# pangsu0613/TransCAR

Measured on AMD Instinct MI355X. Metric: nuScenes frames/sec (6-cam+radar, 900 queries): fusion decoder (Detr3DHead.forward + box decode), FPN features resident in HBM, higher is better.
Workload: dtype f32 (linear steps and attention core of the batched launches: f16x2 split operands, 3 v_mfma_f32_16x16x32_f16 products, fp32 accumulate; activations of the 32-row tiles held as two f16 planes; 4- / 8-row tiles: f32 MFMA)

## Files before the change

### transcar_amd/csrc/chain.hip

```cpp
#include <stdlib.h>
#include <string.h>

#include <type_traits>

#include "kernels.hpp"
#ifdef TC_CHAIN_STAMPS
__device__ long long g_cam_stamps[4][8];
#define CAM_STAMP(slot)                                                                        \
  do {                                                                                         \
    if (blockIdx.x == 100 && (threadIdx.x & 63) == 0)                                          \
      g_cam_stamps[(threadIdx.x >> 6) & 3][(slot)] = __builtin_amdgcn_s_memtime();             \
  } while (0)
#endif
#include "rowdev.hpp"
#define TC_ONCE_LD(p) ldg4_stream(p)
#ifdef TC_CHAIN_DUMP
__device__ float* g_chain_dump;
__device__ long long g_chain_dump_floats;
#endif

namespace tc {

namespace {

// ... 76 lines not shown
  F_CARRY = 4096,
  F_NOT_LAYER0 = 8192,
  F_PRESYNC = 16384
};
enum GSel : short {
  G_NONE = -1, G_HS = 0, G_QK, G_VT, G_INITREF, G_ATTN_O, G_XIN, G_POS, G_CLS, G_KV0, G_KV1, G_KV2,
  G_QF, G_RFEAT, G_COUNT
};

struct StepDesc {
  short kind, wp, wp2, K, N, src, src2, dst, res, act, flags, gsel, gtsel, sync;
};
constexpr StepDesc PROG_DECODER_T[] = {
    {K_LOAD, 0, 0, 0, 0, B_NONE, B_NONE, B_U1, B_NONE, 0, 0, G_ATTN_O, G_NONE, 0},
    {K_LOAD, 0, 0, 0, 0, B_NONE, B_NONE, B_X, B_NONE, 0, 0, G_XIN, G_NONE, 1},
    {K_LINEAR, 1, -1, 256, 256, B_U1, B_NONE, B_U2, B_X, 0, 0, G_NONE, G_NONE, 1},
    {K_LN, 2, -1, 0, 0, B_U2, B_NONE, B_X, B_U1, 0, F_LN_XP, G_NONE, G_NONE, 1},
    {K_LINEAR, 3, -1, 256, N_LOGITS, B_U1, B_NONE, B_L, B_NONE, 0, 0, G_NONE, G_NONE, 0},
    {K_POSENC, 5, 6, 0, 0, B_NONE, B_NONE, B_U2, B_NONE, 0, F_NOT_W0, G_NONE, G_NONE, 1},
    {K_SAMPLE, 0, 0, 0, 0, B_L, B_NONE, B_U3, B_NONE, 0, 0, G_NONE, G_NONE, 1},
    {K_LINEAR, 7, -1, 256, 256, B_U2, B_NONE, B_U1, B_NONE, 0, 0, G_NONE, G_NONE, 1},
    {K_LINEAR, 4, -1, 256, 256, B_U3, B_NONE, B_U2, B_X, 0, 0, G_NONE, G_NONE, 1},
    {K_LN, 9, 8, 0, 0, B_U2, B_U1, B_X, B_NONE, 0, 0, G_NONE, G_NONE, 1},
    {K_LINEAR, 10, -1, 256, 512, B_X, B_NONE, B_A, B_NONE, 1, 0, G_NONE, G_NONE, 1},
    {K_LINEAR, 11, -1, 512, 256, B_A, B_NONE, B_U3, B_X, 0, 0, G_NONE, G_NONE, 1},
    {K_LN, 12, -1, 0, 0, B_U3, B_NONE, B_X, B_U1, 0, F_LN_XP, G_HS, G_NONE, 1},
    {K_LINEAR, 13, -1, 256, 256, B_X, B_NONE, B_U2, B_NONE, 1, 0, G_NONE, G_NONE, 0},
    {K_LINEAR, 16, -1, 256, 512, B_U1, B_NONE, B_NONE, B_NONE, 0, F_SCALEQ | F_SKIP_NONEXT, G_QK, G_NONE, 0},
    {K_LINEAR, 16, -1, 256, 256, B_X, B_NONE, B_NONE, B_NONE, 0, F_WOFF | F_SKIP_NONEXT, G_NONE, G_VT, 1},
    {K_LINEAR, 14, -1, 256, 256, B_U2, B_NONE, B_U3, B_NONE, 1, 0, G_NONE, G_NONE, 0},
    {K_NARROW, 15, -1, 256, N_CODE, B_U3, B_U1, B_L, B_NONE, 0, F_PRESYNC, G_NONE, G_NONE, 1},
    {K_REFUPD, 0, 0, 0, 0, B_L, B_NONE, B_NONE, B_NONE, 0, 0, G_NONE, G_NONE, 0},
    {K_END, 0, 0, 0, 0, 0, 0, 0, 0, 0, 0, 0, 0, 0}};
constexpr StepDesc PROG_PROLOGUE_T[] = {
    {K_LOAD, 0, 0, 0, 0, B_NONE, B_NONE, B_U1, B_NONE, 0, 0, G_POS, G_NONE, 0},
    {K_LOAD, 0, 0, 0, 0, B_NONE, B_NONE, B_X, B_NONE, 0, 0, G_XIN, G_NONE, 1},
    {K_LINEAR, 0, -1, 256, 3, B_U1, B_NONE, B_NONE, B_NONE, 2, 0, G_INITREF, G_NONE, 0},
    {K_LINEAR, 16, -1, 256, 512, B_X, B_U1, B_NONE, B_NONE, 0, F_SCALEQ, G_QK, G_NONE, 0},
    {K_LINEAR, 16, -1, 256, 256, B_X, B_NONE, B_NONE, B_NONE, 0, F_WOFF, G_NONE, G_VT, 0},
    {K_END, 0, 0, 0, 0, 0, 0, 0, 0, 0, 0, 0, 0, 0}};
constexpr StepDesc PROG_RADAR_ENC_T[] = {
    {K_TOKENS, 0, 0, 0, 0, B_NONE, B_NONE, B_A, B_NONE, 0, 0, G_NONE, G_NONE, 1},
    {K_POSENC, 0, 1, 0, 0, B_A, B_NONE, B_U3, B_NONE, 0, 0, G_NONE, G_NONE, 0},
    {K_LINEAR, 4, -1, 36, 64, B_A, B_NONE, B_X, B_NONE, 1, 0, G_NONE, G_NONE, 1},
    {K_LINEAR, 2, -1, 256, 256, B_U3, B_NONE, B_U1, B_NONE, 0, 0, G_NONE, G_NONE, 0},
    {K_LINEAR, 5, -1, 64, 128, B_X, B_NONE, B_U2, B_NONE, 1, 0, G_NONE, G_NONE, 1},
    {K_LINEAR, 6, -1, 128, 256, B_U2, B_NONE, B_X, B_NONE, 1, 0, G_NONE, G_NONE, 1},
    {K_LN, 3, -1, 0, 0, B_U1, B_NONE, B_U2, B_X, 0, F_LN_RELU, G_NONE, G_NONE, 1},
    {K_LINEAR, 7, -1, 256, 512, B_U2, B_NONE, B_NONE, B_NONE, 0, 0, G_KV0, G_NONE, 0},
    {K_LINEAR, 8, -1, 256, 512, B_U2, B_NONE, B_NONE, B_NONE, 0, 0, G_KV1, G_NONE, 0},
    {K_LINEAR, 9, -1, 256, 512, B_U2, B_NONE, B_NONE, B_NONE, 0, 0, G_KV2, G_NONE, 0},
    {K_END, 0, 0, 0, 0, 0, 0, 0, 0, 0, 0, 0, 0, 0}};
constexpr StepDesc PROG_RADAR_ENC_A_T[] = {
    {K_TOKENS, 0, 0, 0, 0, B_NONE, B_NONE, B_A, B_NONE, 0, 0, G_NONE, G_NONE, 1},
    {K_POSENC, 0, 1, 0, 0, B_A, B_NONE, B_U3, B_NONE, 0, 0, G_NONE, G_NONE, 0},
    {K_LINEAR, 4, -1, 36, 64, B_A, B_NONE, B_X, B_NONE, 1, 0, G_NONE, G_NONE, 1},
    {K_LINEAR, 2, -1, 256, 256, B_U3, B_NONE, B_U1, B_NONE, 0, 0, G_NONE, G_NONE, 0},
    {K_LINEAR, 5, -1, 64, 128, B_X, B_NONE, B_U2, B_NONE, 1, 0, G_NONE, G_NONE, 1},
    {K_LINEAR, 6, -1, 128, 256, B_U2, B_NONE, B_X, B_NONE, 1, 0, G_NONE, G_NONE, 1},
    {K_LN, 3, -1, 0, 0, B_U1, B_NONE, B_U2, B_X, 0, F_LN_RELU, G_RFEAT, G_NONE, 1},
    {K_LINEAR, 7, -1, 256, 512, B_U2, B_NONE, B_NONE, B_NONE, 0, 0, G_KV0, G_NONE, 0},
    {K_END, 0, 0, 0, 0, 0, 0, 0, 0, 0, 0, 0, 0, 0}};
constexpr StepDesc PROG_RADAR_ENC_B_T[] = {
    {K_LOAD, 0, 0, 0, 0, B_NONE, B_NONE, B_X, B_NONE, 0, 0, G_RFEAT, G_NONE, 1},
    {K_LINEAR, 8, -1, 256, 512, B_X, B_NONE, B_NONE, B_NONE, 0, 0, G_KV1, G_NONE, 0},
    {K_LINEAR, 9, -1, 256, 512, B_X, B_NONE, B_NONE, B_NONE, 0, 0, G_KV2, G_NONE, 0},
// ... 67 lines not shown
  float qscale; int qpad;
  DropK drop;
  int dbg;
  int tile_rows;
  int matrix_path;
  int last_cls_only;
  const float* ref_in; int ref_mod; float* ref_out; float* box_m;
  CamK cam; unsigned long long* pair_counter;
  const float* pre; const int* premask;
  const float* tokens; int RI, T, pad_mult;
  const float* ref_last; const float* box_in;
  int cen_from_box;
  float rmin[TC_MAX_RADAR_LAYERS], rmax[TC_MAX_RADAR_LAYERS];
  float* all_box; int* hits;
  const int* row_perm;
  float* tape[T_COUNT]; size_t tape_stride; size_t hits_stride;
  DropK rdrop;
  const float* bwd_cxy[TC_MAX_RADAR_LAYERS]; int bwd_ldc[TC_MAX_RADAR_LAYERS];
  const float* bwd_box[TC_MAX_RADAR_LAYERS];
  int* range_status;
  const float* loss_vals;
  float* loss_out;
  const DetAcc* detp;
};
struct ChainK : ChainDev {
  tc_linear pairs[MAX_PAIRS];
  tc_linear gpairs[MAX_PAIRS];
  float* dy[D_COUNT]; size_t dy_stride = 0;
  const float* d_cls = nullptr; const float* d_box = nullptr;
  float* dkv[TC_MAX_RADAR_LAYERS] = {nullptr, nullptr, nullptr};
  size_t w16_delta = 0;
  int npoints = 1;
  int refine = 1;
};

inline bool generic_xattn(const ChainK& k) { return k.npoints > 1 || k.cam.num_levels < 4; }

constexpr int table_steps(int prog) {
  return (prog == PROG_DECODER ? (int)(sizeof(PROG_DECODER_T) / sizeof(StepDesc))
          : prog == PROG_PROLOGUE ? (int)(sizeof(PROG_PROLOGUE_T) / sizeof(StepDesc))
          : prog_is_enc_full(prog) ? (int)(sizeof(PROG_RADAR_ENC_T) / sizeof(StepDesc))
          : prog == PROG_RADAR_ENC_A ? (int)(sizeof(PROG_RADAR_ENC_A_T) / sizeof(StepDesc))
          : prog == PROG_RADAR_ENC_B ? (int)(sizeof(PROG_RADAR_ENC_B_T) / sizeof(StepDesc))
          : prog == PROG_RADAR_BWD ? (int)(sizeof(PROG_RADAR_BWD_T) / sizeof(StepDesc))
                                     : (int)(sizeof(PROG_RADAR_LAYER_T) / sizeof(StepDesc))) - 1;
}
constexpr int rec_cap(int prog) { return table_steps(prog) * ((prog_is_radar(prog) || prog == PROG_RADAR_BWD) ? TC_MAX_RADAR_LAYERS : 1); }
static_assert(sizeof(BWD_STORE) / sizeof(short) == table_steps(PROG_RADAR_BWD), "backward maps follow the step table");
static_assert(sizeof(RADAR_TAPE) / sizeof(short) == table_steps(PROG_RADAR) && sizeof(ENC_TAPE) / sizeof(short) == table_steps(PROG_RADAR_ENC),
              "tape maps follow the step tables");
inline const StepDesc* prog_table(int prog) {
  return prog == PROG_DECODER ? PROG_DECODER_T
         : prog == PROG_PROLOGUE ? PROG_PROLOGUE_T
         : prog_is_enc_full(prog) ? PROG_RADAR_ENC_T
         : prog == PROG_RADAR_ENC_A ? PROG_RADAR_ENC_A_T
         : prog == PROG_RADAR_ENC_B ? PROG_RADAR_ENC_B_T
         : prog == PROG_RADAR_BWD ? PROG_RADAR_BWD_T : PROG_RADAR_LAYER_T;
}

struct LinSpec {
  const float* W; const float* bias; int K, N;
  const float* src; int src_ld;
  const float* src2; int src2_ld;
  float* dst; int dst_ld;
  const float* res; int res_ld;
  const int* gate;
// ... 1852 lines not shown
}

template <int RA, int RB, int PROGB, int MM = 0, bool PRE = false, bool MP = false>
__global__ __launch_bounds__(nw_of(RA) * 64, 2) void chain_dual_kernel(ChainDev ka, ChainDev kb, int na,
                                                           Recs<rec_cap(PROG_DECODER), nw_of(RA)> ra,
                                                           Recs<rec_cap(PROGB), nw_of(RB)> rb) {
  static_assert(nw_of(RA) == nw_of(RB), "both programs of a launch run with the same workgroup size");
  if ((int)blockIdx.x < na) chain_body<RA, PROG_DECODER, false, MM, PRE, MP>(ka, ra.s, blockIdx.x);
  else chain_body<RB, PROGB, false, MM>(kb, rb.s, (int)blockIdx.x - na);
}

template <int R, int PROG>
int lds_off(int id) {
  using Lds = ChainLds<R, rec_cap(PROG)>;
  const int unit0 = (int)(offsetof(Lds, unit) / 4), ustride = R * LD2;
  switch (id) {
    case B_A: return unit0 + ustride;
    case B_X: return unit0;
    case B_U1: return unit0 + ustride;
    case B_U2: return unit0 + 2 * ustride;
    case B_U3: return unit0 + 3 * ustride;
    case B_L: return (int)(offsetof(Lds, l) / 4);
    default: return -1;
  }
}
template <int R, int PROG>
constexpr size_t chain_lds_bytes() { return sizeof(ChainLds<R, rec_cap(PROG)>); }
inline int buf_ld_h(int id) { return id == B_A ? LD5 : id == B_L ? LDL : LD2; }

template <int R, int PROG, int MM = 0>
void resolve_program(ChainK& k, StepAllT<nw_of(R)>* out) {
  constexpr int NW = nw_of(R);
  const StepDesc* table = prog_table(PROG);
  constexpr int nsteps = table_steps(PROG);
  const int nrep = (prog_is_radar(PROG) || PROG == PROG_RADAR_BWD) ? k.nlayers : 1;
  const int total = nsteps * nrep;
  memset(out, 0, sizeof(StepAllT<NW>) * rec_cap(PROG));
  for (int idx = 0; idx < total; ++idx) {
    const int rep = idx / nsteps, si = idx - rep * nsteps;
    const int layer = PROG == PROG_RADAR_BWD ? k.nlayers - 1 - rep : rep;
    const int pair0 = (prog_is_radar(PROG) || PROG == PROG_RADAR_BWD) ? layer * RADAR_PAIRS : 0;
    const StepDesc d = table[si];
    StepRes& r = out[idx].r;
    r.K = d.K; r.N = d.N;
    r.kind = d.kind; r.src = d.src; r.src2 = d.src2; r.dst = d.dst; r.res = d.res; r.act = d.act;
    r.flags = d.flags; r.sync = d.sync; r.rep = (short)rep; r.si = (short)si;
    if ((d.flags & F_SKIP_NONEXT) && !k.has_next) r.kind = K_NOP;
    if (PROG == PROG_DECODER && !k.refine &&
        (d.kind == K_REFUPD || ((d.kind == K_LINEAR || d.kind == K_NARROW) && d.wp >= 13 && d.wp <= 15)))
      r.kind = K_NOP;
    if (PROG == PROG_RADAR && k.last_cls_only && rep + 1 < nrep && d.wp >= 6 && d.wp <= 10 &&
        (d.kind == K_LINEAR || d.kind == K_LN || d.kind == K_NARROW))
      r.kind = K_NOP;
    if (d.gsel != G_NONE) { r.gd = k.g[d.gsel]; r.gld = k.g_ld[d.gsel]; r.gmod = k.g_mod[d.gsel]; }
    if (d.gtsel != G_NONE) r.gt = k.g[d.gtsel];
    bool taped = false;
    if (PROG == PROG_RADAR_TRAIN) {
      if (d.flags & F_SCALEQ) r.flags = (short)(r.flags & ~F_SCALEQ);
      r.flags = (short)(r.flags & ~F_IFHIT);
      if (d.kind == K_LINEAR && d.wp == 4) r.flags = (short)(r.flags | F_GPRE);
      const short ts = RADAR_TAPE[si];
      if (ts != T_NONE && r.gd == nullptr) { r.gd = k.tape[ts] + (size_t)rep * k.tape_stride; r.gld = 256; taped = true; }
    }
    if (PROG == PROG_RADAR_BWD) {
      if ((d.flags & F_NOT_LAYER0) && layer == 0) r.kind = K_NOP;
      const short ds = BWD_STORE[si], ts = BWD_TAPE[si], ts2 = BWD_TAPE2[si];
      if (ds != D_NONE && k.dy[ds] != nullptr) { r.gd = k.dy[ds] + (size_t)layer * k.dy_stride; taped = true; }
// ... 279 lines not shown
  const tc_decoder_layer& w = *a.w;
  const tc_pos_encoder& pe = w.position_encoder;
  k.pairs[0] = w.self_attn.in_proj; k.pairs[1] = w.self_attn.out_proj;
  k.pairs[2] = tc_linear{w.norm0.g, w.norm0.b};
  k.pairs[3] = w.attention_weights; k.pairs[4] = w.output_proj; k.pairs[5] = pe.l0;
  k.pairs[6] = tc_linear{pe.n1.g, pe.n1.b}; k.pairs[7] = pe.l3; k.pairs[8] = tc_linear{pe.n4.g, pe.n4.b};
  k.pairs[9] = tc_linear{w.norm1.g, w.norm1.b}; k.pairs[10] = w.ffn0; k.pairs[11] = w.ffn1;
  k.pairs[12] = tc_linear{w.norm2.g, w.norm2.b};
  k.pairs[13] = w.reg.l0; k.pairs[14] = w.reg.l2; k.pairs[15] = w.reg.l4;
  k.refine = w.reg.l0.w != nullptr;
  TC_REQUIRE(k.refine || a.box_m == nullptr, "decoder_chain: a layer without a reg branch writes no box");
  k.has_next = a.next_in_proj != nullptr;
  if (k.has_next) k.pairs[16] = *a.next_in_proj;
  k.w16_delta = w.packed16_delta;
  k.g[G_ATTN_O] = const_cast<float*>(a.attn_o); k.g_ld[G_ATTN_O] = 256; k.g_mod[G_ATTN_O] = a.attn_mod;
  k.g[G_XIN] = const_cast<float*>(a.x_in); k.g_ld[G_XIN] = a.x_ld; k.g_mod[G_XIN] = a.x_mod;
  k.g[G_POS] = const_cast<float*>(a.qe); k.g_ld[G_POS] = 512; k.g_mod[G_POS] = a.Q;
  k.g[G_HS] = a.hs; k.g_ld[G_HS] = 256;
  k.g[G_QK] = a.qk; k.g_ld[G_QK] = 512; k.g[G_VT] = a.vt;
  k.qscale = a.qscale; k.qpad = a.qpad;
  k.ref_in = a.ref_in; k.ref_mod = a.ref_mod; k.ref_out = a.ref_out; k.box_m = a.box_m;
  fill_camk(a.cam, k.cam);
  k.pair_counter = a.cam.pair_counter;
  TC_REQUIRE((a.pre == nullptr) == (a.premask == nullptr), "decoder_chain: pre-gathered values and masks come together");
  TC_REQUIRE(a.pre == nullptr || a.cam.feats.num_levels == 4,
             "decoder_chain: num_levels=%d (the camera pre-gather exists for 4 levels)", a.cam.feats.num_levels);
  k.pre = a.pre; k.premask = a.premask;
  TC_REQUIRE(a.tile_rows == 0 || a.tile_rows == 4 || a.tile_rows == 8 || a.tile_rows == 16 || a.tile_rows == 32,
             "decoder_chain: tile_rows=%d (0 = automatic, 4, 8, 16 or 32)", a.tile_rows);
  k.tile_rows = a.tile_rows;
  k.matrix_path = a.matrix_path;
  k.drop = a.drop;
  k.range_status = a.range_status;
  return 0;
}

int launch_decoder_chain(const DecoderChainArgs& a, hipStream_t s) {
  ChainK k;
  int rc = make_decoder_k(a, k);
  if (rc != 0) return rc;
  return launch(k, s, "chain(decoder)");
}

static int make_radar_enc_k(const RadarEncodeArgs& a, ChainK& k, int part = 0) {
  TC_REQUIRE(a.RI <= 64 && (a.RI & 3) == 0, "radar_encode: radar_in_dims=%d", a.RI);
  TC_REQUIRE(a.nlayers == TC_MAX_RADAR_LAYERS, "radar_encode: %d radar layers (3 supported)", a.nlayers);
  init_k(k);
  k.program = part == 1 ? PROG_RADAR_ENC_A : part == 2 ? PROG_RADAR_ENC_B : PROG_RADAR_ENC;
  if (a.tape != nullptr) {
    TC_REQUIRE(part == 0, "radar_encode: the training forward runs the whole encoder program");
    k.program = PROG_RADAR_ENC_TRAIN;
    for (int i = 0; i < T_COUNT; ++i) k.tape[i] = a.tape[i];
  }
  k.M = a.M; k.Q = 1; k.RI = a.RI; k.tokens = a.tokens; k.has_next = 1;
  k.w16_delta = a.w16_delta; k.matrix_path = a.matrix_path; k.range_status = a.range_status;
  TC_REQUIRE(part == 0 || a.radar_feat != nullptr, "radar_encode: split programs need the radar_feat buffer");
  k.g[G_RFEAT] = a.radar_feat; k.g_ld[G_RFEAT] = 256;
  k.pairs[0] = a.rpe.l0; k.pairs[1] = tc_linear{a.rpe.n1.g, a.rpe.n1.b}; k.pairs[2] = a.rpe.l3;
  k.pairs[3] = tc_linear{a.rpe.n4.g, a.rpe.n4.b}; k.pairs[4] = a.f0; k.pairs[5] = a.f2; k.pairs[6] = a.f4;
  for (int r = 0; r < TC_MAX_RADAR_LAYERS; ++r) {
    k.pairs[7 + r] = a.kvproj[r];
    k.g[G_KV0 + r] = a.kv[r]; k.g_ld[G_KV0 + r] = 512;
  }
  return 0;
}

int launch_radar_encode(const RadarEncodeArgs& a, hipStream_t s) {
// ... 215 lines not shown
```

### transcar_amd/csrc/head.hip

```cpp
#include <math.h>
#include <stdarg.h>
#include <stdlib.h>
#include <string.h>

#include "kernels.hpp"

namespace tc {

static thread_local char g_err[512] = "";

void set_error(const char* fmt, ...) {
  va_list ap;
  va_start(ap, fmt);
  vsnprintf(g_err, sizeof(g_err), fmt, ap);
  va_end(ap);
}

int check_launch(const char* what) {
  hipError_t e = hipGetLastError();
  if (e != hipSuccess) {
    set_error("%s: %s", what, hipGetErrorString(e));
    return (int)e;
  }
  return 0;
// ... 110 lines not shown
};

static size_t head_ws_layout(const tc_head_weights* w, int B, int T, void* base, size_t cap,
                             HeadWs* out) {
  const int Q = w->num_query, C = w->embed_dims, F = w->ffn_dims, L = w->num_layers;
  const size_t rows = (size_t)B * Q, rt = (size_t)B * T;
  const int qpad = ((Q + 15) / 16) * 16;
  Arena a(base, cap);
  HeadWs h;
  h.qpad = qpad;
  h.pos = a.take<float>(rows * C); h.x = a.take<float>(rows * C);
  h.qk = a.take<float>(rows * 2 * C); h.vt = a.take<float>((size_t)B * C * qpad);
  h.attn_o = a.take<float>(rows * C);
  h.t0 = a.take<float>(rows * C); h.t1 = a.take<float>(rows * C); h.t2 = a.take<float>(rows * C);
  h.ffn_h = a.take<float>(rows * F);
  h.logits = a.take<float>(rows * w->num_cams * w->num_levels * head_points(w));
  h.sampled = a.take<float>(rows * C);
  h.init_ref = a.take<float>(rows * 3); h.inter_refs = a.take<float>((size_t)L * rows * 3);
  h.hs = a.take<float>((size_t)L * rows * C);
  h.reg_tmp = a.take<float>(rows * w->code_size); h.box_m = a.take<float>(rows * w->code_size);
  h.tp0 = a.take<float>(rt * C); h.tp1 = a.take<float>(rt * C);
  h.f0 = a.take<float>(rt * 64); h.f1 = a.take<float>(rt * 128); h.f2 = a.take<float>(rt * C);
  h.radar_feat = a.take<float>(rt * C); h.kv = a.take<float>(rt * 2 * C);
  for (int i = 0; i < TC_MAX_RADAR_LAYERS; ++i) h.kv3[i] = a.take<float>(rt * 2 * C);
  h.qproj = a.take<float>(rows * C); h.rattn = a.take<float>(rows * C);
  h.cxy = a.take<float>(rows * 2); h.addref = a.take<float>(rows * 3);
  h.qf = a.take<float>(rows * C);
  h.hits = a.take<int>((size_t)TC_MAX_RADAR_LAYERS * rows);
  h.perm = a.take<int>(rows); h.hitflag = a.take<int>(rows);
  if (out) *out = h;
  return a.off;
}

static int head_forward_fused(const tc_head_weights* w, const tc_feats_nhwc* feats, int B,
                              const float* lidar2img, float img_h, float img_w,
                              const float* radar_tokens, int T, int pad_mult, float* all_cls_scores,
                              float* all_bbox_preds, const tc_head_aux* aux, const tc_head_options& opt,
                              const HeadWs& h_, hipStream_t s) {
  const int Q = w->num_query, C = w->embed_dims, L = w->num_layers, H = w->num_heads;
  const int code = w->code_size, ncls = w->num_classes;
  const int rows = B * Q, rt = B * T;
  const float attn_qscale = 1.4426950408889634f / sqrtf((float)(C / H));
  HeadWs h = h_;
  if (aux != nullptr) {
    if (aux->inter_states) h.hs = aux->inter_states;
    if (aux->inter_references) h.inter_refs = aux->inter_references;
    if (aux->last_box) h.box_m = aux->last_box;
  }
  unsigned long long* pairs = aux ? aux->sample_pairs : nullptr;
  const bool radar = w->num_radar_layers > 0;
  bool refine = true;
  TC_TRY(decoder_refines(w, &refine));

  const int enc_first = opt.phase != 0 && L > 1 ? L - 2 : 0;
  const int lid_begin = opt.phase == 2 ? enc_first : 0, lid_end = opt.phase == 1 ? enc_first : L;
  RadarEncodeArgs re;
  if (radar) {
    re.tokens = radar_tokens; re.RI = w->radar_in_dims; re.M = rt;
    re.rpe = w->radar_position_encoder; re.f0 = w->radar_feat0; re.f2 = w->radar_feat2;
    re.f4 = w->radar_feat4; re.nlayers = w->num_radar_layers;
    for (int r = 0; r < TC_MAX_RADAR_LAYERS; ++r) {
      const tc_mha& m = w->radar[r].attn;
      re.kvproj[r] = tc_linear{m.in_proj.w ? m.in_proj.w + (size_t)C * C : nullptr,
                               m.in_proj.b ? m.in_proj.b + C : nullptr};
      re.kv[r] = h.kv3[r];
    }
    re.radar_feat = h.radar_feat;
    re.w16_delta = w->packed16_delta; re.matrix_path = opt.matrix_path; re.range_status = opt.range_status;
  }

  const bool ddrop = opt.decoder_dropout_p > 0.0f;
  TC_REQUIRE(!ddrop || (unsigned long long)(opt.dropout_seed_stride ? 1 : B) * H * Q * Q < (1ull << 32),
             "decoder dropout: B*H*Q*Q exceeds 32 bits");
  if (radar && ddrop && opt.phase != 1) TC_TRY(launch_radar_encode(re, s));
  const bool folded = !ddrop && w->l0_attn_out != nullptr && w->l0_init_reference != nullptr;
  if (!folded && opt.phase != 2) {
    PrologueArgs pa;
    pa.qe = w->query_embedding; pa.Q = Q; pa.M = rows; pa.refpts = w->reference_points;
    pa.in_proj = w->layers[0].self_attn.in_proj; pa.init_ref = h.init_ref; pa.qk = h.qk; pa.vt = h.vt;
    pa.qpad = h.qpad; pa.qscale = attn_qscale; pa.w16_delta = w->packed16_delta;
    TC_TRY(launch_prologue(pa, s));
  }
  for (int lid = lid_begin; lid < lid_end; ++lid) {
    const bool l0c = folded && lid == 0;
    const bool init_in = lid == 0 || !refine;
    const float* ref_in = init_in ? (folded ? w->l0_init_reference : h.init_ref)
                                  : h.inter_refs + (size_t)(lid - 1) * rows * 3;
    DecoderChainArgs d;
    if (ddrop) {
      d.drop = make_drop(opt.decoder_dropout_p, opt.dropout_seed, 16u + 8u * (unsigned)lid, 0u);
      if (opt.dropout_seed_stride != 0) { d.drop.seed_stride = opt.dropout_seed_stride; d.drop.rows_per_sample = (unsigned)Q; }
    }
    d.attn_o = l0c ? w->l0_attn_out : h.attn_o;
    d.attn_mod = l0c ? Q : 0; d.ref_mod = folded && init_in ? Q : 0;
    if (lid == 0) { d.x_in = w->query_embedding + C; d.x_ld = 2 * C; d.x_mod = Q; }
    else { d.x_in = h.hs + (size_t)(lid - 1) * rows * C; d.x_ld = C; d.x_mod = 0; }
    d.qe = w->query_embedding; d.Q = Q;
    d.ref_in = ref_in; d.ref_out = h.inter_refs + (size_t)lid * rows * 3;
    d.box_m = lid == L - 1 ? h.box_m : nullptr;
    if (!refine) d.ref_out = h.addref;
    d.w = &w->layers[lid];
    d.next_in_proj = lid + 1 < L ? &w->layers[lid + 1].self_attn.in_proj : nullptr;
    d.qscale = attn_qscale;
    d.hs = h.hs + (size_t)lid * rows * C; d.qk = h.qk; d.vt = h.vt; d.qpad = h.qpad;
    d.cam.feats = *feats; d.cam.B = B; d.cam.Q = Q; d.cam.C = C; d.cam.num_cams = w->num_cams;
    d.cam.num_points = head_points(w);
    d.cam.lidar2img = lidar2img; d.cam.ref = ref_in; d.cam.logits = nullptr;
    for (int i = 0; i < 6; ++i) d.cam.pc[i] = w->pc_range[i];
    d.cam.img_h = img_h; d.cam.img_w = img_w; d.cam.out = nullptr; d.cam.vis = nullptr;
    d.cam.pair_counter = pairs;
    d.code = code; d.M = rows; d.tile_rows = opt.chain_tile_rows; d.matrix_path = opt.matrix_path;
    d.range_status = opt.range_status;
    if (!l0c) {
      const int trows = opt.chain_tile_rows ? opt.chain_tile_rows : (rows <= 1024 ? 4 : rows <= 2048 ? 8 : 16);
      if (trows >= 16 && opt.matrix_path != TC_MATRIX_F32) {
        PreGatherArgs pga;
        const bool pre = !ddrop && opt.cam_pregather == 1;
        if (pre) {
          float* pbuf = static_cast<float*>(opt.cam_pregather_ws);
          int* pmask = reinterpret_cast<int*>(pbuf + (size_t)rows * w->num_cams * w->num_levels * C);
          pga.cam = d.cam; pga.M = rows; pga.ref_mod = d.ref_mod; pga.out = pbuf; pga.mask = pmask;
          d.pre = pbuf; d.premask = pmask;
        }
        TC_TRY(launch_self_attn_core_x(h.qk, h.qk + C, 2 * C, h.vt, h.qpad, h.attn_o, C, B, Q, H, s, ddrop ? &d.drop : nullptr,
                                       pre ? &pga : nullptr));
      } else {
        TC_TRY(launch_self_attn_core(h.qk, h.qk + C, 2 * C, h.vt, h.qpad, h.attn_o, C, B, Q, H, s, ddrop ? &d.drop : nullptr));
      }
    }
    if (radar && !ddrop && lid == enc_first) TC_TRY(launch_decoder_chain_with_encoders(d, re, L > 1 ? 1 : 0, s));
    else if (radar && !ddrop && L > 1 && lid == enc_first + 1) TC_TRY(launch_decoder_chain_with_encoders(d, re, 2, s));
    else TC_TRY(launch_decoder_chain(d, s));
  }
  if (opt.phase == 1) return 0;
  if (!refine)
    TC_TRY(launch_ref_broadcast(folded ? w->l0_init_reference : h.init_ref, folded ? Q : 0, h.inter_refs, rows, L, s));
  if (aux) {
    if (aux->init_reference) {
      if (folded) {
        for (int b = 0; b < B; ++b)
          TC_HIP(hipMemcpyAsync(aux->init_reference + (size_t)b * Q * 3, w->l0_init_reference,
                                (size_t)Q * 3 * 4, hipMemcpyDeviceToDevice, s));
      } else {
        TC_HIP(hipMemcpyAsync(aux->init_reference, h.init_ref, (size_t)rows * 3 * 4, hipMemcpyDeviceToDevice, s));
      }
// ... 398 lines not shown

size_t tc_box_decode_workspace_bytes(int B, int Q, int num_classes) {
  return box_decode_ws_bytes(B, Q, num_classes);
}

int tc_box_decode_topk(const float* cls_scores, const float* bbox_preds, int B, int Q,
                       int num_classes, int code_size, int max_num, const float* post_center_range,
                       float* boxes, float* scores, int* labels, unsigned char* valid,
                       void* workspace, size_t workspace_bytes, tc_stream_t stream) {
  return launch_box_decode(cls_scores, bbox_preds, B, Q, num_classes, code_size, max_num,
                           post_center_range, boxes, scores, labels, valid, workspace,
                           workspace_bytes, as_stream(stream));
}

int tc_box_decode_kept(const float* cls_scores, const float* bbox_preds, int B, int Q, int num_classes, int code_size,
                       int max_num, const float* post_center_range, float score_threshold, int use_threshold,
                       int z_shift, float* kept_boxes, float* kept_scores, long long* kept_labels, int* kept_count,
                       tc_stream_t stream) {
  BoxDecodeKept k{kept_boxes, kept_scores, kept_labels, kept_count, score_threshold, use_threshold, z_shift};
  return launch_box_decode(cls_scores, bbox_preds, B, Q, num_classes, code_size, max_num, post_center_range,
                           nullptr, nullptr, nullptr, nullptr, nullptr, 0, as_stream(stream), &k);
}

size_t tc_head_packed_bytes(const tc_head_weights* w) {
  if (check_dims(w) != 0) return 0;
  bool refine;
  if (decoder_refines(w, &refine) != 0) return 0;
  tc_head_weights view = *w;
  PackItem items[MAX_PACK_ITEMS];
  const int n = collect_pack_items(w, &view, items);
  size_t total = 0;
  for (int i = 0; i < n; ++i)
    if (!items[i].narrow && !items[i].absent) total += 3 * arena_slice(packed_floats(items[i].N, items[i].K), 4);
  const size_t Q = w->num_query, C = w->embed_dims, qpad = ((Q + 15) / 16) * 16;
  total += arena_slice(Q * 3, 4) + arena_slice(Q * C, 4) + arena_slice(Q * 2 * C, 4) + arena_slice(C * qpad, 4);
  return total;
}

int tc_head_pack_weights(const tc_head_weights* w, void* packed, size_t packed_bytes,
                         tc_head_weights* packed_view, tc_stream_t stream) {
  TC_TRY(check_dims(w));
  bool refine;
  TC_TRY(decoder_refines(w, &refine));
  TC_REQUIRE(packed != nullptr && packed_view != nullptr, "pack_weights: null output");
  TC_REQUIRE(packed_bytes >= tc_head_packed_bytes(w), "pack_weights: buffer too small");
  *packed_view = *w;
  PackItem items[MAX_PACK_ITEMS];
  const int n = collect_pack_items(w, packed_view, items);
  Arena a(packed, packed_bytes);
  size_t region_a = 0;
  for (int i = 0; i < n; ++i)
    if (!items[i].narrow && !items[i].absent) region_a += arena_slice(packed_floats(items[i].N, items[i].K), 4);
  const size_t delta = region_a / sizeof(float);
  for (int i = 0; i < n; ++i) {
    if (items[i].absent) { *items[i].slot = nullptr; continue; }
    TC_REQUIRE(items[i].src != nullptr, "pack_weights: weight %d is null", i);
    if (items[i].narrow) continue;
    float* dst = a.take<float>(packed_floats(items[i].N, items[i].K));
    TC_TRY(launch_pack_linear(items[i].src, items[i].N, items[i].K, dst, dst + delta, dst + 2 * delta, as_stream(stream)));
    *items[i].slot = dst;
  }
  for (int rgn = 0; rgn < 2; ++rgn)
    for (int i = 0; i < n; ++i)
      if (!items[i].narrow && !items[i].absent) a.take<float>(packed_floats(items[i].N, items[i].K));
  packed_view->packed16_delta = delta;
  for (int l = 0; l < TC_MAX_LAYERS; ++l) packed_view->layers[l].packed16_delta = delta;
  for (int l = 0; l < TC_MAX_RADAR_LAYERS; ++l) packed_view->radar[l].packed16_delta = delta;
  {
    const int Q = w->num_query, C = w->embed_dims, H = w->num_heads;
    const int qpad = ((Q + 15) / 16) * 16;
    float* init_ref = a.take<float>((size_t)Q * 3);
    float* attn_o = a.take<float>((size_t)Q * C);
    float* qk = a.take<float>((size_t)Q * 2 * C);
    float* vt = a.take<float>((size_t)C * qpad);
    hipStream_t s = as_stream(stream);
    TC_HIP(hipMemsetAsync(vt, 0, (size_t)C * qpad * 4, s));
    PrologueArgs pa;
    pa.qe = w->query_embedding; pa.Q = Q; pa.M = Q; pa.refpts = packed_view->reference_points;
    pa.in_proj = packed_view->layers[0].self_attn.in_proj; pa.init_ref = init_ref; pa.qk = qk; pa.vt = vt;
    pa.qpad = qpad; pa.qscale = 1.4426950408889634f / sqrtf((float)(C / H));
    pa.w16_delta = delta;
    TC_TRY(launch_prologue(pa, s));
    TC_TRY(launch_self_attn_core(qk, qk + C, 2 * C, vt, qpad, attn_o, C, 1, Q, H, s));
    packed_view->l0_init_reference = init_ref;
    packed_view->l0_attn_out = attn_o;
  }
  return 0;
}

int tc_head_repack_trainable_ex(const tc_head_weights* w, tc_head_weights* packed_view, int copies,
                                tc_stream_t stream) {
  TC_TRY(check_dims(w));
  TC_REQUIRE(packed_view != nullptr && packed_view->l0_attn_out != nullptr,
             "repack_trainable: packed_view was not produced by tc_head_pack_weights");
  TC_REQUIRE(copies == 1 || copies == 3, "repack_trainable: copies=%d (1: the 4x4x1 copy, 3: both)", copies);
  tc_head_weights scratch = *packed_view;
  PackItem items[MAX_PACK_ITEMS];
  const int n = collect_pack_items(w, &scratch, items);
  const int first = 1 + 10 * w->num_layers;
  PackJob jobs[MAX_PACK_ITEMS];
  int nj = 0;
  for (int i = first; i < n; ++i) {
    TC_REQUIRE(items[i].src != nullptr, "repack_trainable: weight %d is null", i);
    if (items[i].narrow) continue;
    float* dst = const_cast<float*>(*items[i].slot);
    jobs[nj] = PackJob{items[i].src, dst, copies == 3 ? dst + packed_view->packed16_delta : nullptr,
                       items[i].N, items[i].K};
    jobs[nj++].PH = copies == 3 ? dst + 2 * packed_view->packed16_delta : nullptr;
  }
  if (nj == 0) return 0;
  return launch_pack_group(jobs, nj, as_stream(stream));
}

extern "C" int radar_train_transposed_jobs(const tc_head_weights* w, int B, int T, void* workspace, size_t workspace_bytes,
                                           tc::PackJob* jobs, int cap);

int tc_radar_train_repack(const tc_head_weights* w, tc_head_weights* packed_view, void* bwd_workspace,
                          size_t bwd_workspace_bytes, int B, int T, tc_stream_t stream) {
// ... 284 lines not shown
```

### transcar_amd/csrc/kernels.hpp

```cpp
#pragma once
#include "common.hpp"
#include "../../include/transcar_hip.h"

namespace tc {

struct GemmArgs {
  const float* X = nullptr;  int ldx = 0;
  const float* X2 = nullptr; int x2_cols = 0;
  const float* W = nullptr;  int ldw = 0;
  const float* bias = nullptr;
  const float* R = nullptr;  int ldr = 0;
  const int* rowgate = nullptr;
  float* Y = nullptr;        int ldy = 0;
  float* Yt = nullptr;
  int t_col0 = 0, t_ld = 0, t_rows_per_batch = 1;
  int M = 0, K = 0, N = 0;
  int act = 0;
  float scale = 1.0f; int scale_cols = 0;
};
int launch_gemm(const GemmArgs& a, hipStream_t s);

struct LnArgs {
  const float* a = nullptr;
  const float* b = nullptr;
// ... 33 lines not shown
  int B, Q, C, num_cams;
  const float* lidar2img; const float* ref; const float* logits;
  float pc[6]; float img_h, img_w;
  float* out; unsigned char* vis; unsigned long long* pair_counter;
  int num_points = 1;
};
int launch_cam_sample(const CamSampleArgs& a, hipStream_t s);

struct PrologueArgs {
  const float* qe; int Q, M;
  tc_linear refpts, in_proj;
  float* init_ref; float* qk; float* vt; int qpad; float qscale;
  size_t w16_delta = 0;
};
int launch_prologue(const PrologueArgs& a, hipStream_t s);

struct DecoderChainArgs {
  const float* attn_o;
  int attn_mod = 0, ref_mod = 0;
  const float* x_in; int x_ld, x_mod;
  const float* qe; int Q;
  const float* ref_in; float* ref_out; float* box_m;
  const tc_decoder_layer* w;
  const tc_linear* next_in_proj;
  float qscale;
  float* hs; float* qk; float* vt; int qpad;
  CamSampleArgs cam;
  int code, M;
  int tile_rows = 0;
  int matrix_path = 0;
  DropK drop = DropK{0, 0, 1.0f, 0, 0, 0, 0, 0};
  int* range_status = nullptr;
  const float* pre = nullptr; const int* premask = nullptr;
};
int launch_decoder_chain(const DecoderChainArgs& a, hipStream_t s);

struct RadarEncodeArgs {
  const float* tokens; int RI, M;
  tc_pos_encoder rpe; tc_linear f0, f2, f4;
  int nlayers; tc_linear kvproj[TC_MAX_RADAR_LAYERS]; float* kv[TC_MAX_RADAR_LAYERS];
  float* radar_feat;
  size_t w16_delta = 0;
  float* const* tape = nullptr;
  int matrix_path = 0;
  int* range_status = nullptr;
};
int launch_radar_encode(const RadarEncodeArgs& a, hipStream_t s);
int launch_decoder_chain_with_encoders(const DecoderChainArgs& d, const RadarEncodeArgs& e, int part,
                                       hipStream_t s);

struct RadarChainArgs {
  const float* qf; const float* ref_last; const float* box_m;
  const float* tokens; int RI;
  const float* kv[TC_MAX_RADAR_LAYERS];
  tc_radar_layer w[TC_MAX_RADAR_LAYERS];
  int nlayers, Q, T, pad_mult, code, ncls, M;
  float qscale; float pc[6];
  float* all_cls; float* all_box; int* hits;
  int tile_rows = 0;
  int matrix_path = 0;
  int last_cls_only = 0;
  int cen_from_box = 0;
  const int* row_perm = nullptr;
  float* const* tape = nullptr; size_t tape_stride = 0, hits_stride = 0;
  DropK drop = DropK{0, 0, 1.0f, 0, 1500, 0, 0, 0};
  int* range_status = nullptr;
};
enum DySlot { DY_DBOX = 0, DY_DT1, DY_DT0, DY_DC2, DY_DC0, DY_DFF, DY_DH, DY_DPROJ, DY_DQP, DY_DCLS, DY_COUNT };
// ... 115 lines not shown
```

Baseline: 10270.

## Precompute input-independent layer-0 decoder stages at weight-pack time

At weight-packing time this runs the parts of decoder layer 0 that depend only on weights and the learned query embedding: the self-attention output projection, its layer norm, the query positional encoding and the value-side linear. Results are stored as constant planes for each tile-size and matrix-path variant. At forward time a shortened layer-0 step table loads these planes and skips the matching linear, layer-norm and posenc steps. This removes repeated per-frame work that does not depend on the input, at the cost of more packed-weight memory and a separate code path restricted to eval mode with one point and four levels.

```diff
diff --git a/transcar_amd/csrc/chain.hip b/transcar_amd/csrc/chain.hip
--- a/transcar_amd/csrc/chain.hip
+++ b/transcar_amd/csrc/chain.hip
@@ -132,6 +132,35 @@
     {K_NARROW, 15, -1, 256, N_CODE, B_U3, B_U1, B_L, B_NONE, 0, F_PRESYNC, G_NONE, G_NONE, 1},
     {K_REFUPD, 0, 0, 0, 0, B_L, B_NONE, B_NONE, B_NONE, 0, 0, G_NONE, G_NONE, 0},
     {K_END, 0, 0, 0, 0, 0, 0, 0, 0, 0, 0, 0, 0, 0}};
+constexpr StepDesc PROG_DECODER_L0_T[] = {
+    {K_LOAD, 0, 0, 0, 0, B_NONE, B_NONE, B_U1, B_NONE, 0, 0, G_ATTN_O, G_NONE, 0},
+    {K_LOAD, 0, 0, 0, 0, B_NONE, B_NONE, B_U2, B_NONE, 0, 0, G_KV1, G_NONE, 0},
+    {K_LOAD, 0, 0, 0, 0, B_NONE, B_NONE, B_X, B_NONE, 0, 0, G_XIN, G_NONE, 1},
+    {K_LINEAR, 3, -1, 256, N_LOGITS, B_U1, B_NONE, B_L, B_NONE, 0, 0, G_NONE, G_NONE, 0},
+    {K_POSENC, 5, 6, 0, 0, B_NONE, B_NONE, B_U3, B_NONE, 0, F_NOT_W0, G_NONE, G_NONE, 1},
+    {K_SAMPLE, 0, 0, 0, 0, B_L, B_NONE, B_U3, B_NONE, 0, 0, G_NONE, G_NONE, 1},
+    {K_LINEAR, 4, -1, 256, 256, B_U3, B_NONE, B_U1, B_X, 0, 0, G_NONE, G_NONE, 1},
+    {K_LN, 9, 8, 0, 0, B_U1, B_U2, B_X, B_NONE, 0, 0, G_NONE, G_NONE, 1},
+    {K_LINEAR, 10, -1, 256, 512, B_X, B_NONE, B_A, B_NONE, 1, 0, G_NONE, G_NONE, 1},
+    {K_LINEAR, 11, -1, 512, 256, B_A, B_NONE, B_U3, B_X, 0, 0, G_NONE, G_NONE, 1},
+    {K_LN, 12, -1, 0, 0, B_U3, B_NONE, B_X, B_U1, 0, F_LN_XP, G_HS, G_NONE, 1},
+    {K_LINEAR, 13, -1, 256, 256, B_X, B_NONE, B_U2, B_NONE, 1, 0, G_NONE, G_NONE, 0},
+    {K_LINEAR, 16, -1, 256, 512, B_U1, B_NONE, B_NONE, B_NONE, 0, F_SCALEQ | F_SKIP_NONEXT, G_QK, G_NONE, 0},
+    {K_LINEAR, 16, -1, 256, 256, B_X, B_NONE, B_NONE, B_NONE, 0, F_WOFF | F_SKIP_NONEXT, G_NONE, G_VT, 1},
+    {K_LINEAR, 14, -1, 256, 256, B_U2, B_NONE, B_U3, B_NONE, 1, 0, G_NONE, G_NONE, 0},
+    {K_NARROW, 15, -1, 256, N_CODE, B_U3, B_U1, B_L, B_NONE, 0, F_PRESYNC, G_NONE, G_NONE, 1},
+    {K_REFUPD, 0, 0, 0, 0, B_L, B_NONE, B_NONE, B_NONE, 0, 0, G_NONE, G_NONE, 0},
+    {K_END, 0, 0, 0, 0, 0, 0, 0, 0, 0, 0, 0, 0, 0}};
+constexpr StepDesc PROG_DECODER_L0GEN_T[] = {
+    {K_LOAD, 0, 0, 0, 0, B_NONE, B_NONE, B_U1, B_NONE, 0, 0, G_ATTN_O, G_NONE, 0},
+    {K_LOAD, 0, 0, 0, 0, B_NONE, B_NONE, B_X, B_NONE, 0, 0, G_XIN, G_NONE, 1},
+    {K_LINEAR, 1, -1, 256, 256, B_U1, B_NONE, B_U2, B_X, 0, 0, G_NONE, G_NONE, 1},
+    {K_LN, 2, -1, 0, 0, B_U2, B_NONE, B_X, B_U1, 0, F_LN_XP, G_KV0, G_NONE, 1},
+    {K_POSENC, 5, 6, 0, 0, B_NONE, B_NONE, B_U2, B_NONE, 0, F_NOT_W0, G_NONE, G_NONE, 1},
+    {K_LINEAR, 7, -1, 256, 256, B_U2, B_NONE, B_U1, B_NONE, 0, 0, G_KV1, G_NONE, 1},
+    {K_END, 0, 0, 0, 0, 0, 0, 0, 0, 0, 0, 0, 0, 0}};
+static_assert(sizeof(PROG_DECODER_L0_T) <= sizeof(PROG_DECODER_T) && sizeof(PROG_DECODER_L0GEN_T) <= sizeof(PROG_DECODER_T),
+              "the layer-0 sequences fit the decoder program's records");
 constexpr StepDesc PROG_PROLOGUE_T[] = {
     {K_LOAD, 0, 0, 0, 0, B_NONE, B_NONE, B_U1, B_NONE, 0, 0, G_POS, G_NONE, 0},
     {K_LOAD, 0, 0, 0, 0, B_NONE, B_NONE, B_X, B_NONE, 0, 0, G_XIN, G_NONE, 1},
@@ -265,6 +294,7 @@
   size_t w16_delta = 0;
   int npoints = 1;
   int refine = 1;
+  int l0_seq = 0;
 };
 
 inline bool generic_xattn(const ChainK& k) { return k.npoints > 1 || k.cam.num_levels < 4; }
@@ -2183,7 +2213,11 @@
 void resolve_program(ChainK& k, StepAllT<nw_of(R)>* out) {
   constexpr int NW = nw_of(R);
   const StepDesc* table = prog_table(PROG);
-  constexpr int nsteps = table_steps(PROG);
+  int nsteps = table_steps(PROG);
+  if (PROG == PROG_DECODER && k.l0_seq != 0) {
+    table = k.l0_seq == 1 ? PROG_DECODER_L0_T : PROG_DECODER_L0GEN_T;
+    nsteps = (int)((k.l0_seq == 1 ? sizeof(PROG_DECODER_L0_T) : sizeof(PROG_DECODER_L0GEN_T)) / sizeof(StepDesc)) - 1;
+  }
   const int nrep = (prog_is_radar(PROG) || PROG == PROG_RADAR_BWD) ? k.nlayers : 1;
   const int total = nsteps * nrep;
   memset(out, 0, sizeof(StepAllT<NW>) * rec_cap(PROG));
@@ -2529,7 +2563,51 @@
   k.matrix_path = a.matrix_path;
   k.drop = a.drop;
   k.range_status = a.range_status;
+  if (a.l0_consts != nullptr) {
+    TC_REQUIRE(!generic_xattn(k) && k.drop.thr == 0 && a.pre == nullptr,
+               "decoder_chain: layer-0 constants exist for the eval-mode one-point, four-level kernels");
+    const size_t plane = decoder_l0_const_floats(a.Q) / 3;
+    k.l0_seq = 1;
+    k.g[G_XIN] = const_cast<float*>(a.l0_consts); k.g_ld[G_XIN] = 256; k.g_mod[G_XIN] = a.Q;
+    k.g[G_ATTN_O] = const_cast<float*>(a.l0_consts) + plane; k.g_ld[G_ATTN_O] = 256; k.g_mod[G_ATTN_O] = a.Q;
+    k.g[G_KV1] = const_cast<float*>(a.l0_consts) + 2 * plane; k.g_ld[G_KV1] = 256; k.g_mod[G_KV1] = a.Q;
+  }
   return 0;
+}
+
+size_t decoder_l0_const_floats(int Q) { return 3 * (arena_slice((size_t)Q * 256, 4) / 4); }
+
+int decoder_l0_variant(int M, int tile_rows_opt, int matrix_path) {
+  ChainK k;
+  init_k(k);
+  k.M = M; k.tile_rows = tile_rows_opt; k.matrix_path = matrix_path;
+  const int rows = tile_rows(k);
+  return rows == 4 ? 0 : rows == 8 ? 1 : rows == 32 ? 4 : use_f16x2(k) ? 3 : 2;
+}
+
+__global__ void l0_xpos_kernel(const float* __restrict__ x, const float* __restrict__ qe, float* __restrict__ xp, int n) {
+  const int i = blockIdx.x * blockDim.x + threadIdx.x;
+  if (i < n) xp[i] = __fadd_rn(x[i], qe[(size_t)(i >> 8) * 512 + (i & 255)]);
+}
+
+int launch_decoder_l0_consts(const DecoderChainArgs& a, int variant, float* consts, hipStream_t s) {
+  static const int rows_of[TC_L0_VARIANTS] = {4, 8, 16, 16, 32};
+  static const int path_of[TC_L0_VARIANTS] = {TC_MATRIX_F32, TC_MATRIX_F32, TC_MATRIX_F32, TC_MATRIX_F16X2, TC_MATRIX_F16X2};
+  TC_REQUIRE(variant >= 0 && variant < TC_L0_VARIANTS && a.M == a.Q, "decoder_l0_consts: variant=%d M=%d Q=%d", variant, a.M, a.Q);
+  ChainK k;
+  int rc = make_decoder_k(a, k);
+  if (rc != 0) return rc;
+  TC_REQUIRE(!generic_xattn(k) && k.drop.thr == 0, "decoder_l0_consts: one-point, four-level eval-mode kernels only");
+  const size_t plane = decoder_l0_const_floats(a.Q) / 3;
+  k.l0_seq = 2; k.has_next = 0;
+  k.tile_rows = rows_of[variant]; k.matrix_path = path_of[variant];
+  k.g[G_KV0] = consts; k.g_ld[G_KV0] = 256;
+  k.g[G_KV1] = consts + 2 * plane; k.g_ld[G_KV1] = 256;
+  rc = launch(k, s, "chain(layer-0 constants)");
+  if (rc != 0) return rc;
+  const int n = a.Q * 256;
+  hipLaunchKernelGGL(l0_xpos_kernel, dim3((n + 255) / 256), dim3(256), 0, s, consts, a.qe, consts + plane, n);
+  return check_launch("l0_xpos");
 }
 
 int launch_decoder_chain(const DecoderChainArgs& a, hipStream_t s) {
diff --git a/transcar_amd/csrc/head.hip b/transcar_amd/csrc/head.hip
--- a/transcar_amd/csrc/head.hip
+++ b/transcar_amd/csrc/head.hip
@@ -166,6 +166,18 @@
   return a.off;
 }
 
+static bool l0_foldable(const tc_head_weights* w) { return head_points(w) == 1 && w->num_levels == TC_MAX_LEVELS; }
+static size_t l0_scratch_bytes(const tc_head_weights* w) {
+  const size_t Q = w->num_query, C = w->embed_dims, qpad = ((Q + 15) / 16) * 16;
+  const size_t scratch = arena_slice(Q * 2 * C, 4) + arena_slice(C * qpad, 4);
+  const size_t consts = l0_foldable(w) ? TC_L0_VARIANTS * decoder_l0_const_floats((int)Q) * sizeof(float) : 0;
+  return consts > scratch ? consts : scratch;
+}
+static const float* l0_consts_of(const tc_head_weights* packed_view, int variant) {
+  const size_t Q = packed_view->num_query, C = packed_view->embed_dims;
+  return packed_view->l0_attn_out + arena_slice(Q * C, 4) / sizeof(float) + (size_t)variant * decoder_l0_const_floats((int)Q);
+}
+
 static int head_forward_fused(const tc_head_weights* w, const tc_feats_nhwc* feats, int B,
                               const float* lidar2img, float img_h, float img_w,
                               const float* radar_tokens, int T, int pad_mult, float* all_cls_scores,
@@ -208,6 +220,7 @@
              "decoder dropout: B*H*Q*Q exceeds 32 bits");
   if (radar && ddrop && opt.phase != 1) TC_TRY(launch_radar_encode(re, s));
   const bool folded = !ddrop && w->l0_attn_out != nullptr && w->l0_init_reference != nullptr;
+  const int l0_variant = folded && l0_foldable(w) ? decoder_l0_variant(rows, opt.chain_tile_rows, opt.matrix_path) : -1;
   if (!folded && opt.phase != 2) {
     PrologueArgs pa;
     pa.qe = w->query_embedding; pa.Q = Q; pa.M = rows; pa.refpts = w->reference_points;
@@ -245,6 +258,7 @@
     d.cam.pair_counter = pairs;
     d.code = code; d.M = rows; d.tile_rows = opt.chain_tile_rows; d.matrix_path = opt.matrix_path;
     d.range_status = opt.range_status;
+    if (l0c && l0_variant >= 0) d.l0_consts = l0_consts_of(w, l0_variant);
     if (!l0c) {
       const int trows = opt.chain_tile_rows ? opt.chain_tile_rows : (rows <= 1024 ? 4 : rows <= 2048 ? 8 : 16);
       if (trows >= 16 && opt.matrix_path != TC_MATRIX_F32) {
@@ -709,8 +723,8 @@
   size_t total = 0;
   for (int i = 0; i < n; ++i)
     if (!items[i].narrow && !items[i].absent) total += 3 * arena_slice(packed_floats(items[i].N, items[i].K), 4);
-  const size_t Q = w->num_query, C = w->embed_dims, qpad = ((Q + 15) / 16) * 16;
-  total += arena_slice(Q * 3, 4) + arena_slice(Q * C, 4) + arena_slice(Q * 2 * C, 4) + arena_slice(C * qpad, 4);
+  const size_t Q = w->num_query, C = w->embed_dims;
+  total += arena_slice(Q * 3, 4) + arena_slice(Q * C, 4) + l0_scratch_bytes(w);
   return total;
 }
 
@@ -761,6 +775,18 @@
     TC_TRY(launch_self_attn_core(qk, qk + C, 2 * C, vt, qpad, attn_o, C, 1, Q, H, s));
     packed_view->l0_init_reference = init_ref;
     packed_view->l0_attn_out = attn_o;
+    if (l0_foldable(w)) {
+      static_assert(sizeof(float) == 4, "slices are counted in floats");
+      DecoderChainArgs d{};
+      d.attn_o = attn_o; d.x_in = w->query_embedding + C; d.x_ld = 2 * C; d.x_mod = Q;
+      d.qe = w->query_embedding; d.Q = Q; d.ref_in = init_ref;
+      d.w = &packed_view->layers[0]; d.qscale = pa.qscale; d.qpad = qpad;
+      d.cam.feats.num_levels = w->num_levels; d.cam.B = 1; d.cam.Q = Q; d.cam.C = C; d.cam.num_cams = w->num_cams;
+      d.cam.num_points = 1; d.cam.ref = init_ref;
+      d.code = w->code_size; d.M = Q;
+      for (int v = 0; v < TC_L0_VARIANTS; ++v)
+        TC_TRY(launch_decoder_l0_consts(d, v, const_cast<float*>(l0_consts_of(packed_view, v)), s));
+    }
   }
   return 0;
 }
diff --git a/transcar_amd/csrc/kernels.hpp b/transcar_amd/csrc/kernels.hpp
--- a/transcar_amd/csrc/kernels.hpp
+++ b/transcar_amd/csrc/kernels.hpp
@@ -89,8 +89,13 @@
   DropK drop = DropK{0, 0, 1.0f, 0, 0, 0, 0, 0};
   int* range_status = nullptr;
   const float* pre = nullptr; const int* premask = nullptr;
+  const float* l0_consts = nullptr;
 };
 int launch_decoder_chain(const DecoderChainArgs& a, hipStream_t s);
+constexpr int TC_L0_VARIANTS = 5;
+size_t decoder_l0_const_floats(int Q);
+int decoder_l0_variant(int M, int tile_rows, int matrix_path);
+int launch_decoder_l0_consts(const DecoderChainArgs& a, int variant, float* consts, hipStream_t s);
 
 struct RadarEncodeArgs {
   const float* tokens; int RI, M;
```

Result: faster. 10390 (median of 6 runs) (+1.2%).
